# segeschecho/OpenEKFMonoSLAM

Hardware: AMD Instinct MI355X
Metric: EKF updates/s (frames/s) at N features (higher is better)
Workload: dtype f32 storage; i8 MFMA with exact i32 sums (downdate) + f64 (B, S, state)

## Files before the change

### openekfmonoslam_amd/csrc/engine.cpp

```cpp
#include "engine.h"
#include "../../include/ekf_test_hooks.h"

#include <cmath>
#include <cstdio>
#include <algorithm>
#include <atomic>
#include <cstdlib>
#include <chrono>
#include <cstring>
#include <mutex>
#include <new>

#include <dlfcn.h>
#include <rccl/rccl.h>

using namespace ekf;

namespace ekf {
void launch_partition(EkfEngine *e, const EkfMatch *src, int M, const uint8_t *flags, EkfMatch *dst1, EkfMatch *dst0,
                      int *cnt1, bool map_update = false, const uint8_t *d_kdesc = nullptr, int *d_idx0 = nullptr,
                      int publish_seq = 0, bool rescue = false);
void launch_outlier_idx(EkfEngine *e, const EkfMatch *src, int M, int *idx);
}

// ... 573 lines not shown
            if (sharded) {
                sym.resize((size_t)cnt * n);
                for (int i = 0; i < cnt; ++i)
                    for (int j = 0; j < n; ++j) {
                        const double a = P[(size_t)(g0 + i) * n + j], c = P[(size_t)j * n + g0 + i];
                        sym[(size_t)i * n + j] = e->f32 ? (double)(0.5f * (float)a + 0.5f * (float)c) : 0.5 * a + 0.5 * c;
                    }
                src = sym.data();
            }
            uint8_t *dst = (uint8_t *)e->d.P + (size_t)l0 * e->ldP * w;
            if (e->f32) {
                tmp.resize((size_t)cnt * n);
                for (size_t i = 0; i < (size_t)cnt * n; ++i) tmp[i] = (float)src[i];
                HIPCHK(hipMemcpy2D(dst, (size_t)e->ldP * 4, tmp.data(), (size_t)n * 4, (size_t)n * 4, cnt, hipMemcpyHostToDevice));
            } else {
                HIPCHK(hipMemcpy2D(dst, (size_t)e->ldP * 8, src, (size_t)n * 8, (size_t)n * 8, cnt, hipMemcpyHostToDevice));
            }
        }
        e->p_exact_sym = sharded;
    }
    HIPCHK(hipMemset(e->d.pred_vis, 0, (size_t)e->cap * sizeof(int)));
    HIPCHK(hipMemset(e->d.pred_vis_full, 0, (size_t)e->cap * sizeof(int)));
    e->n_step_preds = 0;
    HIPCHK(hipMemset(e->d.feat_times_predicted, 0, (size_t)e->cap * sizeof(unsigned)));
    HIPCHK(hipMemset(e->d.feat_times_matched, 0, (size_t)e->cap * sizeof(unsigned)));
    return EKF_OK;
}

int ekf_get_state(EkfEngine *e, double x13[13], double *feature_pos, double *P)
{
    if (!e) return EKF_ERR_INVALID_ARG;
    HIPCHK(hipSetDevice(e->device));
    HIPCHK(hipStreamSynchronize(e->stream));
    const int pending = take_pending_error(e);
    if (x13) HIPCHK(hipMemcpy(x13, e->d.state, 13 * sizeof(double), hipMemcpyDeviceToHost));
    if (feature_pos && e->N > 0)
        HIPCHK(hipMemcpy(feature_pos, e->d.feat_pos, (size_t)6 * e->N * sizeof(double), hipMemcpyDeviceToHost));
    if (P) {
        const int n = e->n;
        const size_t w = e->f32 ? 4 : 8;
        const bool sharded = e->shard_world > 1;
        const int blocks[2][3] = {{0, sharded ? 13 : n, 0}, {e->rm.r0, sharded ? e->rm.r1 - e->rm.r0 : 0, e->rm.base}};
        std::vector<float> tmp;
        for (const auto &b : blocks) {
            const int g0 = b[0], cnt = b[1], l0 = b[2];
            if (cnt <= 0) continue;
// ... 108 lines not shown
    HIPCHK(hipSetDevice(e->device));
    HIPCHK(hipStreamSynchronize(e->stream));
    HIPCHK(hipMemcpy(preds, e->d.step_preds, (size_t)e->n_step_preds * sizeof(EkfPrediction), hipMemcpyDeviceToHost));
    return EKF_OK;
}

int ekf_get_feature_layout(EkfEngine *e, int32_t *type, int32_t *covpos)
{
    if (!e) return EKF_ERR_INVALID_ARG;
    for (int i = 0; i < e->N; ++i) {
        if (type) type[i] = e->h_type[i];
        if (covpos) covpos[i] = e->h_covpos[i];
    }
    return EKF_OK;
}

int ekf_add_features(EkfEngine *e, const double *uv, const uint8_t *desc32, int count)
{
    if (!e || count < 0 || (count > 0 && !uv)) return EKF_ERR_INVALID_ARG;
    if (count == 0) return EKF_OK;
    NOT_WHEN_SHARDED(e)
    if (e->N + count > e->cap) return EKF_ERR_CAPACITY;
    HIPCHK(hipSetDevice(e->device));
    double *d_uv = e->d.mm_scratch, *d_Jpo = d_uv + 2 * (size_t)e->cap, *d_Jhr = d_Jpo + 42 * (size_t)count;
    HIPCHK(hipMemcpyAsync(d_uv, uv, (size_t)2 * count * sizeof(double), hipMemcpyHostToDevice, e->stream));
    uint8_t *dd = e->d.feat_desc + (size_t)e->N * e->desc_bytes;
    if (desc32) HIPCHK(hipMemcpyAsync(dd, desc32, (size_t)count * e->desc_bytes, hipMemcpyHostToDevice, e->stream));
    else HIPCHK(hipMemsetAsync(dd, 0, (size_t)count * e->desc_bytes, e->stream));
    HIPCHK(hipMemsetAsync(e->d.feat_times_predicted + e->N, 0, (size_t)count * 4, e->stream));
    HIPCHK(hipMemsetAsync(e->d.feat_times_matched + e->N, 0, (size_t)count * 4, e->stream));
    launch_add_features(e, d_uv, count, d_Jpo, d_Jhr);
    for (int j = 0; j < count; ++j) {
        e->h_type.push_back(EKF_FEATURE_INVERSE_DEPTH);
        e->h_covpos.push_back(e->n + 6 * j);
    }
    e->N += count;
    e->n += 6 * count;
    e->n_pred = 0;
    refresh_row_map(e);
    HIPCHK(hipStreamSynchronize(e->stream));
    return check_async(e);
}

static int compact_map(EkfEngine *e, const std::vector<uint8_t> &drop_feature, const std::vector<uint8_t> &drop_row)
{
    NOT_WHEN_SHARDED(e)
// ... 40 lines not shown
        return EKF_ERR_INVALID_ARG;
    }
    if (w > 0) {
        HIPCHK(hipMemcpy(e->d.feat_pos, pos.data(), (size_t)6 * w * 8, hipMemcpyHostToDevice));
        HIPCHK(hipMemcpy(e->d.feat_desc, desc.data(), (size_t)w * e->desc_bytes, hipMemcpyHostToDevice));
        HIPCHK(hipMemcpy(e->d.tmpl, tmpl.data(), (size_t)w * 363, hipMemcpyHostToDevice));
        HIPCHK(hipMemcpy(e->d.feat_times_predicted, tp.data(), (size_t)w * 4, hipMemcpyHostToDevice));
        HIPCHK(hipMemcpy(e->d.feat_times_matched, tm.data(), (size_t)w * 4, hipMemcpyHostToDevice));
        HIPCHK(hipMemcpy(e->d.feat_type, e->h_type.data(), (size_t)w * 4, hipMemcpyHostToDevice));
        HIPCHK(hipMemcpy(e->d.feat_covpos, e->h_covpos.data(), (size_t)w * 4, hipMemcpyHostToDevice));
    }
    e->N = w;
    e->n = n_new;
    refresh_row_map(e);
    e->n_pred = 0;
    return check_async(e);
}

int ekf_remove_features(EkfEngine *e, const int32_t *feat_idx, int count)
{
    if (!e || count < 0 || (count > 0 && !feat_idx)) return EKF_ERR_INVALID_ARG;
    if (count == 0) return EKF_OK;
    HIPCHK(hipSetDevice(e->device));
    std::vector<uint8_t> df(e->N, 0), dr(e->n, 0);
    for (int i = 0; i < count; ++i) {
        const int f = feat_idx[i];
        if (f < 0 || f >= e->N || (i > 0 && feat_idx[i] <= feat_idx[i - 1])) return EKF_ERR_INVALID_ARG;
        df[f] = 1;
        for (int k = 0; k < dims_of(e->h_type[f]); ++k) dr[e->h_covpos[f] + k] = 1;
    }
    return compact_map(e, df, dr);
}

int ekf_remove_bad_features(EkfEngine *e, int *n_removed)
{
    if (!e) return EKF_ERR_INVALID_ARG;
    HIPCHK(hipSetDevice(e->device));
    HIPCHK(hipStreamSynchronize(e->stream));
    const int N = e->N;
    std::vector<unsigned> tp(N), tm(N);
    if (N > 0) {
        HIPCHK(hipMemcpy(tp.data(), e->d.feat_times_predicted, (size_t)N * 4, hipMemcpyDeviceToHost));
        HIPCHK(hipMemcpy(tm.data(), e->d.feat_times_matched, (size_t)N * 4, hipMemcpyDeviceToHost));
    }
    std::vector<int32_t> idx;
    for (int i = 0; i < N; ++i) {
        const float pct = static_cast<float>(tm[i]) / static_cast<float>(tp[i]);
        if (pct < e->cfg.par.goodFeatureMatchingPercent) idx.push_back(i);
    }
    if (n_removed) *n_removed = (int)idx.size();
    return ekf_remove_features(e, idx.data(), (int)idx.size());
}

int ekf_convert_inverse_depth_to_depth(EkfEngine *e, int *converted_index)
{
    if (!e) return EKF_ERR_INVALID_ARG;
    if (converted_index) *converted_index = -1;
    if (e->N == 0) return EKF_OK;
    NOT_WHEN_SHARDED(e)
    HIPCHK(hipSetDevice(e->device));
    double *d_li = e->d.mm_scratch;
    launch_linearity(e, d_li);
    std::vector<double> li(e->N);
    HIPCHK(hipMemcpyAsync(li.data(), d_li, (size_t)e->N * 8, hipMemcpyDeviceToHost, e->stream));
    HIPCHK(hipStreamSynchronize(e->stream));
    int fi = -1;
    for (int i = 0; i < e->N; ++i)
        if (e->h_type[i] == EKF_FEATURE_INVERSE_DEPTH && li[i] < e->cfg.par.inverseDepthLinearityIndexThreshold) {
            fi = i;
            break;
        }
    if (fi < 0) return EKF_OK;
    const int pos = e->h_covpos[fi];
    double *d_J = e->d.mm_scratch + e->cap, *d_T3 = d_J + 32;
    launch_convert(e, fi, pos, d_J, d_T3);
    e->h_type[fi] = EKF_FEATURE_DEPTH;
    std::vector<uint8_t> df(e->N, 0), dr(e->n, 0);
    dr[pos + 3] = dr[pos + 4] = dr[pos + 5] = 1;
    if (converted_index) *converted_index = fi;
    return compact_map(e, df, dr);
}

constexpr int POLL_SECONDS = 20;
// ... 35 lines not shown
            for (int i = 0; i < CNT_COUNT; ++i) e->h_counts[i] = m[i];
            return EKF_OK;
        }
        if ((spin & 0xfffff) == 0xfffff &&
            ((hipStreamQuery(e->stream) == hipSuccess && m[CNT_COUNT] != seq) || std::chrono::steady_clock::now() > t_end)) break;
#if defined(__x86_64__)
        __builtin_ia32_pause();
#endif
    }
    return read_counts(e);
}

static int check_async(EkfEngine *e)
{
    HIPCHK(hipGetLastError());
    return EKF_OK;
}

int ekf_predict(EkfEngine *e)
{
    if (!e) return EKF_ERR_INVALID_ARG;
    HIPCHK(hipSetDevice(e->device));
    launch_predict(e);
    return check_async(e);
}

static int complete_hp_table(EkfEngine *e)
{
    if (e->shard_world <= 1 || e->hp_complete) return EKF_OK;
    int rc;
    std::vector<int32_t> rb(e->shard_world + 1);
    for (int r = 0; r <= e->shard_world; ++r) rb[r] = 2 * e->shard_feat_begin[r];
    if ((rc = exchange_rows(e, EKF_XCHG_HP, e->d.HP, (size_t)e->ldP * hp_elem_bytes(e), rb, "the H.P row blocks"))) return rc;
    if (e->f32 && !e->exact && (rc = exchange_rows(e, EKF_XCHG_HPC, e->d.HPc, 16 * sizeof(double), rb, "the fp64 camera columns of H.P"))) return rc;
    e->hp_complete = true;
    return EKF_OK;
}

static int predict_measurements_dev(EkfEngine *e, const int *d_idx, int count, int *n_out, bool count_predicted = false,
                                    bool lean = false)
{
    launch_predict_features(e, d_idx, d_idx ? count : e->N, false);
    const bool slots = lean && !d_idx && e->shard_world > 1;
    if (slots) launch_shard_bounds_idx(e, e->d.plist, e->d.counts + CNT_NPRED);
    int rc = read_counts(e);
    if (rc) return rc;
    const int np = e->h_counts[d_idx ? CNT_NPRED_SUB : CNT_NPRED];
    if (slots) {
        e->slot_rb.assign(e->shard_world + 1, 0);
        for (int r = 0; r <= e->shard_world; ++r) e->slot_rb[r] = e->h_counts[CNT_SHARD0 + r];
    } else if (!d_idx) e->slot_rb.clear();
    launch_hp_rows(e, d_idx ? e->d.plist_sub : e->d.plist, np, count_predicted);
    if (!d_idx) e->n_pred = np;
    *n_out = np;
    if (e->shard_world > 1 && np > 0) {
        e->hp_complete = false;
        if (!lean && (rc = complete_hp_table(e))) return rc;
        std::vector<int32_t> rb(e->shard_world + 1);
        for (int r = 0; r <= e->shard_world; ++r) rb[r] = e->shard_feat_begin[r];
        if ((rc = exchange_rows(e, EKF_XCHG_PRED_S, e->d.pred_S, 4 * sizeof(double), rb, "the innovation covariance blocks"))) return rc;
    }
    if (!d_idx && e->keep_step_preds) {
        launch_pack_predictions(e, e->d.plist, np, e->d.step_preds);
        e->n_step_preds = np;
    }
    if (!d_idx && e->img.valid) {
        launch_gate_snapshot(e, np);
        e->n_gates = np;
    }
    return check_async(e);
}

static int download_predictions(EkfEngine *e, const int *d_list, int np, EkfPrediction *preds, double *Hs, double *Hf)
{
    if (np <= 0) return EKF_OK;
// ... 183 lines not shown
    int rc = validate_matches(e, matches, M);
    if (rc) return rc;
    if (n_hypotheses) *n_hypotheses = 0;
    if (M == 0) return EKF_OK;
    HIPCHK(hipSetDevice(e->device));
    HIPCHK(hipMemcpyAsync(e->d.matches, matches, (size_t)M * sizeof(EkfMatch), hipMemcpyHostToDevice, e->stream));
    if ((rc = complete_hp_table(e))) return rc;
    rc = ransac_dev(e, M);
    if (rc) return rc;
    HIPCHK(hipMemcpy(inlier_mask, e->d.best_flags, (size_t)M, hipMemcpyDeviceToHost));
    if (n_hypotheses) *n_hypotheses = e->h_counts[CNT_RS_NEXT];
    return EKF_OK;
}

static int lean_gather_exchange(EkfEngine *e, int M)
{
    (void)M;
    int rc;
    if ((rc = exchange_rows(e, EKF_XCHG_HP, e->d.G, (size_t)e->ldP * hp_elem_bytes(e), e->shard_rb, "the gathered H.P rows"))) return rc;
    if (e->f32 && !e->exact && (rc = exchange_rows(e, EKF_XCHG_HPC, e->d.Gc, 16 * sizeof(double), e->shard_rb, "their fp64 camera columns"))) return rc;
    return EKF_OK;
}

static int update_dev(EkfEngine *e, int M, bool update_cov, bool lean = false)
{
    if (M <= 0) return EKF_OK;
    lean = lean && e->shard_world > 1 && !e->hp_complete;
    if (lean) {
        launch_shard_bounds(e, e->d.msel, M);
        int rc = read_counts(e);
        if (rc) return rc;
        e->shard_rb.assign(e->shard_world + 1, 0);
        for (int r = 0; r <= e->shard_world; ++r) e->shard_rb[r] = 2 * e->h_counts[CNT_SHARD0 + r];
        if (e->shard_rb[0] != 0 || e->shard_rb[e->shard_world] != 2 * M) {
            e->err = "sharded update: the match list is not in feature order";
            return EKF_ERR_INVALID_ARG;
        }
    }
    EkfMatch *save = e->d.matches;
    e->d.matches = e->d.msel;
    e->after_gather = lean ? lean_gather_exchange : nullptr;
    launch_update(e, M, update_cov);
    e->after_gather = nullptr;
    e->d.matches = save;
    if (e->hook_rc) return e->hook_rc;
    return check_async(e);
}

static int recover_failed_update(EkfEngine *e, int *status)
// ... 160 lines not shown
static int detect_step_keypoints(EkfEngine *e);

static int step_dev(EkfEngine *e, const EkfKeypoint *d_kps, const uint8_t *d_desc, int n_kp, EkfStepInfo *info,
                    bool use_ncc = false, bool detect = false)
{
    const bool dev_counts = !use_ncc && !detect && !e->img.valid && !e->keep_step_preds && e->shard_world == 1;
    const bool lean = e->shard_world > 1;
    int *cnt = e->d.counts;
    EkfStepInfo li;
    std::memset(&li, 0, sizeof(li));
    int status = EKF_OK, rc;
    const int retries0 = e->sweep_retries;
    if (!dev_counts && e->err_unread) {
        if ((rc = read_counts(e))) return rc;
        if ((rc = recover_failed_update(e, &status))) return rc;
    }
    bool restarted = false;
restart:
    StageTimer tm(e);
    tm.mark();
    int np = 0;
    if (dev_counts) {
        const bool deferred = launch_predict_with_features(e, e->N);
        launch_hp_rows(e, e->d.plist, e->N, true, cnt + CNT_NPRED, deferred);
    } else {
        launch_predict(e);
        if ((rc = predict_measurements_dev(e, nullptr, e->N, &np, true, lean))) return rc;
    }
    tm.mark();
    int M = 0;
    if (dev_counts) {
        launch_match(e, d_kps, d_desc, e->N, n_kp, cnt + CNT_NPRED, true);
    } else {
        if (detect && (rc = detect_step_keypoints(e))) return rc;
        if (lean) rc = match_sharded_dev(e, use_ncc, d_kps, d_desc, n_kp, &M);
        else rc = use_ncc ? match_ncc_dev(e, &M) : match_dev(e, d_kps, d_desc, n_kp, &M, detect ? cnt + CNT_KP_FOUND : nullptr);
        if (rc) return rc;
    }
    tm.mark();
    if (dev_counts) {
        const int batch = e->cfg.ransac_batch;
        const int seq_r = next_publish_seq(e);
        launch_ransac_batch(e, e->N, 0, batch, cnt + CNT_NMATCH, seq_r);
        if ((rc = wait_counts(e, seq_r))) return rc;
        if (e->h_counts[CNT_ERR] && !restarted) {
            if ((rc = recover_failed_update(e, &status))) return rc;
            restarted = true;
// ... 3 lines not shown
        M = e->h_counts[CNT_NMATCH];
        for (int h0 = batch, nb = batch * RANSAC_WIDE_FACTOR; !e->h_counts[CNT_RS_DONE] && h0 < M; h0 += nb) {
            launch_ransac_batch(e, M, h0, nb);
            if ((rc = read_counts(e))) return rc;
        }
    } else if (M > 0 && (rc = ransac_dev(e, M, lean))) {
        return rc;
    }
    li.n_predicted = np;
    li.n_matches = M;
    int ni = 0, no = 0;
    if (M > 0) {
        li.n_hypotheses = e->h_counts[CNT_RS_NEXT];
        ni = e->h_counts[CNT_RS_BEST];
        no = M - ni;
        launch_partition(e, e->d.matches, M, e->d.best_flags, e->d.msel, e->d.mout, nullptr, true, d_desc, e->d.work_idx);
    }
    li.n_inliers = ni;
    li.n_outliers = no;
    tm.mark();
    if ((rc = update_dev(e, ni, true, lean))) return rc;
    tm.mark();
    int nr = 0;
    if (no > 0) {
        int nop = 0;
        for (int attempt = 0; attempt < 2; ++attempt) {
            if (dev_counts) {
                launch_predict_features(e, e->d.work_idx, no, false);
                launch_hp_rows(e, e->d.plist_sub, no, false, cnt + CNT_NPRED_SUB);
                const int seq_p = next_publish_seq(e);
                launch_partition(e, e->d.mout, no, e->d.mask, e->d.msel, nullptr, cnt + CNT_NRESC, true, d_desc, nullptr, seq_p, true);
                rc = wait_counts(e, seq_p);
            } else {
                rc = predict_measurements_dev(e, e->d.work_idx, no, &nop, false, lean);
            }
            if (rc) return rc;
            if (!e->h_counts[CNT_ERR]) break;
            if ((rc = recover_failed_update(e, &status))) return rc;
        }
        if (dev_counts) {
            nr = e->h_counts[CNT_NRESC];
        } else if (nop > 0) {
            launch_rescue(e, e->d.mout, no);
            launch_partition(e, e->d.mout, no, e->d.mask, e->d.msel, nullptr, cnt + CNT_NRESC, true, d_desc);
            if ((rc = read_counts(e))) return rc;
            nr = e->h_counts[CNT_NRESC];
        }
    }
    li.n_rescued = nr;
    tm.mark();
    if ((rc = update_dev(e, nr, true, lean))) return rc;
    tm.mark();
    if (dev_counts && e->async_errors) {
        e->err_unread = true;
    } else {
        if ((rc = read_counts(e))) return rc;
        if (detect) {
            e->step_kp_detected = e->h_counts[CNT_KP_FOUND];
            e->step_kp_kept = std::min(e->step_kp_detected, e->kcap);
        }
        if ((rc = recover_failed_update(e, &status))) return rc;
    }
    tm.finish();
    li.status = status;
    li.n_sweep_retries = e->sweep_retries - retries0;
    if (info) *info = li;
    return status;
}

int ekf_set_async_errors(EkfEngine *e, int on)
{
    if (!e) return EKF_ERR_INVALID_ARG;
    e->async_errors = on != 0;
    return EKF_OK;
// ... 589 lines not shown
```

### openekfmonoslam_amd/csrc/engine.h

```cpp
#pragma once
#include <hip/hip_runtime.h>

#include <atomic>
#include <cstdint>
#include <map>
#include <memory>
#include <mutex>
#include <string>
#include <vector>

#include "../../include/ekf_engine.h"
#include "device_math.h"

namespace ekf {

constexpr int NB = 32;
constexpr int LD_ALIGN = 128;
constexpr int B_SWEEP_MAX = 2048;
constexpr int DX_SPLIT = 16;
constexpr int RANSAC_WIDE_FACTOR = 8;
#ifndef PX_S_VALUE
#define PX_S_VALUE 5
#endif
constexpr int PX_S = PX_S_VALUE;
// ... 154 lines not shown
};

}

struct EkfEngine {
    EkfEngineConfig cfg;
    ekf::CamD cam;
    ekf::ParD par;
    int device = 0;
    int cap = 0, ncap = 0, mcap = 0, kcap = 0;
    int ldP = 0, ldS = 0, ldW = 0;
    int N = 0, n = 0;
    bool f32 = false;
    bool exact = false;
    int desc_bytes = EKF_DESC_BYTES;
    bool desc_f32 = false;
    int shard_rank = 0, shard_world = 1;
    int p_rows_cap = 0;
    ekf::RowMap rm{13, 13, 13};
    std::vector<int> shard_feat_begin;
    EkfExchangeFn xchg = nullptr;
    void *comm = nullptr;
    bool hp_complete = true;
    int (*after_gather)(EkfEngine *, int) = nullptr;
    int (*exchange_hook)(EkfEngine *, int what, void *base, size_t row_bytes, const std::vector<int32_t> &rb, const char *name) = nullptr;
    std::vector<int32_t> shard_row_begin;
    long long xchg_bytes_planes = 0;
    int hook_rc = 0;
    std::vector<int32_t> shard_rb;
    std::vector<int32_t> slot_rb;
    std::vector<int32_t> last_col_rb;
    void *xchg_user = nullptr;
    int n_cus = 256;
    int b_path = 0;
    int sweep_mode = 2;
    unsigned ps_epoch = 0;
    int ps_fault = 0;
    std::shared_ptr<ekf::SweepRegistry> ps_reg;
    int force_launches = 0;
    int sweep_retries = 0;
    int ps_backoff = 0, ps_backoff_len = 0, ps_ok_streak = 0;
    int last_update_M = 0;
    bool last_update_cov = true;
    bool last_update_sym = false;
    bool last_update_persist = false;
    int ps_cap[2] = {0, 0};
// ... 79 lines not shown
    int x = c;
#pragma unroll
    for (int o = 1; o < 64; o <<= 1) {
        const int y = __shfl_up(x, o, 64);
        if (lane >= o) x += y;
    }
    if (lane == 63) wtot[wv] = x;
    __syncthreads();
    int base = 0, tot = 0;
#pragma unroll
    for (int w = 0; w < 16; ++w) {
        const int t = wtot[w];
        base += w < wv ? t : 0;
        tot += t;
    }
    *total = tot;
    return base + x - c;
}
#endif

void launch_predict(EkfEngine *e);
bool launch_predict_features(EkfEngine *e, const int *d_idx, int count, bool state_only, bool defer_compact = false);
bool launch_predict_with_features(EkfEngine *e, int count);
void launch_hp_rows(EkfEngine *e, const int *d_list, int n_list, bool count_predicted = false, const int *d_count = nullptr, bool from_flags = false);
void launch_match(EkfEngine *e, const EkfKeypoint *kps, const uint8_t *kdesc, int n_pred, int n_kp, const int *d_npred = nullptr,
                  bool with_ransac_init = false, const int *d_nkp = nullptr);
void launch_match_index(EkfEngine *e, int M, const int *d_M = nullptr);
void launch_shard_bounds(EkfEngine *e, const EkfMatch *list, int count);
void launch_shard_bounds_idx(EkfEngine *e, const int *list, const int *d_count);
void launch_match_slots(EkfEngine *e, const EkfKeypoint *kps, const uint8_t *kdesc, int n_kp, int s_lo, int s_hi);
void launch_match_ncc_slots(EkfEngine *e, int s_lo, int s_hi);
void launch_match_compact(EkfEngine *e, const EkfKeypoint *kps, int n_pred);
void launch_match_compact_slots(EkfEngine *e, int n_pred, const EkfKeypoint *d_slot_xy);
void launch_ransac_hyp(EkfEngine *e, int M, int h0, int batch, const int *d_M, int h_lo, int h_hi);
void launch_ransac_select(EkfEngine *e, int M, int h0, int batch, const int *d_M, int publish_seq);
void launch_ransac_batch(EkfEngine *e, int M, int h0, int batch, const int *d_M = nullptr, int publish_seq = 0);
void launch_ransac_init(EkfEngine *e, int M);
void launch_update(EkfEngine *e, int M, bool update_cov);
void launch_p_update_exact(EkfEngine *e, int m, bool use_bc, bool exps_ready = false, bool planes_ready = false);
void launch_round_P_f32(EkfEngine *e);
void launch_diag_extract(EkfEngine *e, float *diag);
void launch_planes_move(EkfEngine *e, bool pack, int m_k, int c_lo, int c_hi, int skip_lo, int skip_hi);
void launch_dx_planes(EkfEngine *e, int m_k);
void launch_slice_columns(EkfEngine *e, int m, int c_lo, int c_hi);
void launch_b_gemm_planes(EkfEngine *e, int m, int c_lo, int c_hi);
void launch_rescue(EkfEngine *e, const EkfMatch *matches, int M);
void launch_state_only_predict(EkfEngine *e, EkfPrediction *d_out);
// ... 33 lines not shown
```

### openekfmonoslam_amd/csrc/kernels_predict.hip

```cpp
#include "engine.h"

namespace ekf {

__device__ void predict_prepare_serial(double *st, double *sG);

__global__ void __launch_bounds__(256) k_predict_prepare(double *st, ParD par, const int *counts)
{
    __shared__ double sG[13 * 6];
    if (filter_frozen(counts)) return;
    const double dt = 1.0;
    const double ln = par.linearAccelSD * par.linearAccelSD * dt * dt;
    const double an = par.angularAccelSD * par.angularAccelSD * dt * dt;
    if (blockIdx.x != 0) return;
    if (threadIdx.x == 0) predict_prepare_serial(st, sG);
    __syncthreads();
    if (threadIdx.x < 169) {
        const int i = threadIdx.x / 13, j = threadIdx.x % 13;
        double s = 0.0;
        for (int k = 0; k < 6; ++k) s += (sG[i * 6 + k] * (k < 3 ? ln : an)) * sG[j * 6 + k];
        st[ST_GQG + i * 13 + j] = s;
    }
}

__device__ void predict_prepare_serial(double *st, double *sG)
// ... 247 lines not shown
        return false;
    }
    int *list = sub ? e->d.plist_sub : e->d.plist, *cnt = e->d.counts + (sub ? CNT_NPRED_SUB : CNT_NPRED);
#define PF_ARGS(L_, C_) e->d.state, e->cam, e->d.feat_pos, e->d.feat_type, d_idx, count, e->d.work_flag, state_only ? e->d.pred_vis2 : e->d.pred_vis, \
                        state_only ? e->d.pred_uv2 : e->d.pred_uv, state_only ? nullptr : e->d.Hs, state_only ? nullptr : e->d.Hf,                      \
                        sub ? nullptr : e->d.pred_vis_full, L_, C_
    if (count <= 256) {
        k_predict_features<256><<<1, 256, 0, e->stream>>>(PF_ARGS(list, cnt));
        return false;
    }
    const int nb = (count + 255) / 256;
    k_predict_features<256><<<nb, 256, 0, e->stream>>>(PF_ARGS(nullptr, nullptr));
#undef PF_ARGS
    if (defer_compact && !sub && !d_idx) return true;
    k_compact<<<1, 1024, 0, e->stream>>>(e->d.work_flag, d_idx, count, sub ? e->d.plist_sub : e->d.plist,
                                         e->d.counts + (sub ? CNT_NPRED_SUB : CNT_NPRED));
    return false;
}

template <typename T, typename TO>
__global__ void __launch_bounds__(256)
k_hp_rows(const T *P, int ld, int n, const int *list, const int *feat_type, const int *feat_covpos,
          const double *Hs_tab, const double *Hf_tab, TO *HP, double *S_tab, RowMap rm, double *HPc, unsigned *times_predicted,
          const int *d_count, const int *flag, int n_items, int *list_out, int *count_out, const int *counts)
{
    const int tid = threadIdx.x;
    if (flag) {
        if ((int)blockIdx.x == n_items) {
            if (blockIdx.y != 0) return;
            __shared__ int wtot[16];
            if (tid < 16) wtot[tid] = 0;
            __syncthreads();
            const int per = (n_items + 255) / 256;
            const int b = tid * per, e = min(n_items, b + per);
            int c = 0;
            for (int i = b; i < e; ++i) c += flag[i] ? 1 : 0;
            int total;
            int pos = block_exclusive_scan_1024(c, wtot, &total);
            for (int i = b; i < e; ++i)
                if (flag[i]) list_out[pos++] = i;
            if (tid == 0) *count_out = total;
            return;
        }
        if (!flag[blockIdx.x]) return;
    } else if (d_count && (int)blockIdx.x >= *d_count) return;
    __shared__ double sH[26];
    __shared__ double sHP[2][13];
    const int fi = flag ? (int)blockIdx.x : list[blockIdx.x];
    const int d = feat_dim(feat_type[fi]);
    const int pos = feat_covpos[fi];
    const bool first = blockIdx.y == 0;
    if (times_predicted && tid == 0 && first && !filter_frozen(counts)) times_predicted[fi]++;
    if (!owns_row(rm, pos)) return;
    const T *Pf = P + (size_t)local_row(rm, pos) * ld;
    if (tid < 14) sH[tid] = Hs_tab[14 * fi + tid];
    else if (tid < 26) sH[tid] = Hf_tab[12 * fi + tid - 14];
    double pcol[13];
    int jcol = -1;
    if (first && tid >= 64 && tid < 64 + 7 + d) {
        jcol = tid - 64 < 7 ? tid - 64 : pos + (tid - 64 - 7);
#pragma unroll
        for (int a = 0; a < 6; ++a) pcol[a] = a < d ? (double)Pf[(size_t)a * ld + jcol] : 0.0;
#pragma unroll
        for (int a = 0; a < 7; ++a) pcol[6 + a] = (double)P[(size_t)a * ld + jcol];
    }
    __syncthreads();
    if (jcol >= 0) {
        double a0 = 0.0, a1 = 0.0, b0 = 0.0, b1 = 0.0;
#pragma unroll
        for (int a = 0; a < 6; ++a)
            if (a < d) {
                a0 += sH[14 + a] * pcol[a];
                a1 += sH[20 + a] * pcol[a];
            }
#pragma unroll
        for (int a = 0; a < 7; ++a) {
            b0 += sH[a] * pcol[6 + a];
            b1 += sH[7 + a] * pcol[6 + a];
        }
        sHP[0][tid - 64] = a0 + b0;
        sHP[1][tid - 64] = a1 + b1;
    }
    TO *o0 = HP + (size_t)(2 * fi) * ld;
    TO *o1 = o0 + ld;
    constexpr int VW = 16 / sizeof(T);
    typedef T vec_t __attribute__((ext_vector_type(VW)));
    const int jb = ((int)blockIdx.y * 256 + tid) * VW;
    if (jb < n) {
        vec_t pf[6], pc[7];
#pragma unroll
        for (int a = 0; a < 6; ++a)
            if (a < d) pf[a] = *(const vec_t *)(Pf + (size_t)a * ld + jb);
#pragma unroll
        for (int a = 0; a < 7; ++a) pc[a] = *(const vec_t *)(P + (size_t)a * ld + jb);
        typedef TO ovec_t __attribute__((ext_vector_type(VW)));
        ovec_t r0, r1;
#pragma unroll
        for (int v = 0; v < VW; ++v) {
            const int j = jb + v;
            double a0 = 0.0, a1 = 0.0;
#pragma unroll
            for (int a = 0; a < 6; ++a)
                if (a < d) {
                    const double p = (double)pf[a][v];
                    a0 += sH[14 + a] * p;
                    a1 += sH[20 + a] * p;
                }
            double b0 = 0.0, b1 = 0.0;
#pragma unroll
            for (int a = 0; a < 7; ++a) {
                const double p = (double)pc[a][v];
// ... 9 lines not shown
                HPc[(size_t)(2 * fi + 1) * 16 + j] = a1;
            }
        }
        if (jb + VW <= n) {
            *(ovec_t *)(o0 + jb) = r0;
            *(ovec_t *)(o1 + jb) = r1;
        } else {
#pragma unroll
            for (int v = 0; v < VW; ++v)
                if (jb + v < n) { o0[jb + v] = r0[v]; o1[jb + v] = r1[v]; }
        }
    }
    if (!first) return;
    __syncthreads();
    if (tid < 4) {
        const int r = tid >> 1, c = tid & 1;
        double s1 = 0.0, s2 = 0.0;
        for (int a = 0; a < 7; ++a) s1 += sHP[r][a] * sH[c * 7 + a];
        for (int a = 0; a < d; ++a) s2 += sHP[r][7 + a] * sH[14 + c * 6 + a];
        S_tab[4 * fi + tid] = s1 + s2 + (r == c ? 1.0 : 0.0);
    }
}

void launch_hp_rows(EkfEngine *e, const int *d_list, int n_list, bool count_predicted, const int *d_count, bool from_flags)
{
    unsigned *tp = count_predicted ? e->d.feat_times_predicted : nullptr;
    if (n_list <= 0) return;
    const int chunks_f = (e->n + 256 * 4 - 1) / (256 * 4), chunks_d = (e->n + 256 * 2 - 1) / (256 * 2);
    const int *flag = from_flags ? e->d.work_flag : nullptr;
    int *lo = from_flags ? e->d.plist : nullptr, *co = from_flags ? e->d.counts + CNT_NPRED : nullptr;
    const int gx = n_list + (from_flags ? 1 : 0);
    if (e->exact && e->f32)
        k_hp_rows<float, double><<<dim3(gx, chunks_f), 256, 0, e->stream>>>((const float *)e->d.P, e->ldP, e->n, d_list, e->d.feat_type,
                                                        e->d.feat_covpos, e->d.Hs, e->d.Hf, (double *)e->d.HP,
                                                        e->d.pred_S, e->rm, e->d.HPc, tp, d_count, flag, n_list, lo, co, e->d.counts);
    else if (e->f32)
        k_hp_rows<float, float><<<dim3(gx, chunks_f), 256, 0, e->stream>>>((const float *)e->d.P, e->ldP, e->n, d_list, e->d.feat_type,
                                                        e->d.feat_covpos, e->d.Hs, e->d.Hf, (float *)e->d.HP,
                                                        e->d.pred_S, e->rm, e->d.HPc, tp, d_count, flag, n_list, lo, co, e->d.counts);
    else
        k_hp_rows<double, double><<<dim3(gx, chunks_d), 256, 0, e->stream>>>((const double *)e->d.P, e->ldP, e->n, d_list,
                                                         e->d.feat_type, e->d.feat_covpos, e->d.Hs, e->d.Hf,
                                                         (double *)e->d.HP, e->d.pred_S, e->rm, e->d.HPc, tp, d_count, flag, n_list, lo, co, e->d.counts);
}

__global__ void __launch_bounds__(256)
k_pack_predictions(const int *list, const int *count, const double *uv_tab, const double *S_tab, EkfPrediction *out,
                   int with_S)
{
    const int k = blockIdx.x * 256 + threadIdx.x;
    if (k >= *count) return;
    const int fi = list[k];
    EkfPrediction p;
    p.featureIndex = fi;
    p._pad = 0;
    p.imagePos[0] = uv_tab[2 * fi];
    p.imagePos[1] = uv_tab[2 * fi + 1];
    for (int i = 0; i < 4; ++i) p.covarianceMatrix[i] = with_S ? S_tab[4 * fi + i] : 0.0;
    out[k] = p;
}

__global__ void __launch_bounds__(256)
k_pack_predictions_n(const int *list, int n, const double *uv_tab, const double *S_tab, EkfPrediction *out)
{
    const int k = blockIdx.x * 256 + threadIdx.x;
    if (k >= n) return;
// ... 25 lines not shown
```

### openekfmonoslam_amd/csrc/kernels_ransac.hip

```cpp
#include "engine.h"

namespace ekf {

constexpr int HYP_THREADS = 512;

template <typename T>
__global__ void __launch_bounds__(HYP_THREADS)
k_ransac_hyp(const double *st, CamD cam, double thr, const double *feat_pos, const int *feat_type,
             const int *feat_covpos, int N, const T *HP, int ld, const double *uv_tab, const double *S_tab,
             const EkfMatch *matches, int M, const int *match_of_feat, int h0, int *hyp_count, uint8_t *hyp_flags,
             int mcap, const int *d_M, int h_lo, int h_hi)
{
    __shared__ double sx[13], sRt[9], sRinv[9], sw[2];
    __shared__ int s_cnt[HYP_THREADS / 64];
    if (d_M) M = *d_M;
    const int h = h0 + blockIdx.x;
    if (h >= M) return;
    if (h < h_lo || h >= h_hi) return;
    const int tid = threadIdx.x;
    const int fi = matches[h].featureIndex;
    const T *g0 = HP + (size_t)(2 * fi) * ld;
    const T *g1 = g0 + ld;
    if (tid == 0) {
        double S[4] = {S_tab[4 * fi] - 1.0 + cam.pixelErrorX, S_tab[4 * fi + 1], S_tab[4 * fi + 2],
                       S_tab[4 * fi + 3] - 1.0 + cam.pixelErrorX};
        double Si[4];
        inv2(S, Si);
        const double ax = matches[h].imagePos[0] - uv_tab[2 * fi];
        const double ay = matches[h].imagePos[1] - uv_tab[2 * fi + 1];
        const double n0 = fabs(ax) > EKF_DELTA ? ax : 0.0;
        const double n1 = fabs(ay) > EKF_DELTA ? ay : 0.0;
        const double w0 = Si[0] * n0 + Si[1] * n1;
        const double w1 = Si[2] * n0 + Si[3] * n1;
        sw[0] = w0;
        sw[1] = w1;
        double x[13];
        for (int i = 0; i < 13; ++i) {
            const double dx = (double)g0[i] * w0 + (double)g1[i] * w1;
            x[i] = st[ST_X + i] + (fabs(dx) > EKF_DELTA ? dx : 0.0);
            sx[i] = x[i];
        }
        double R[9];
        quat_to_rot(x + 3, R);
        for (int i = 0; i < 3; ++i)
            for (int j = 0; j < 3; ++j) sRt[j * 3 + i] = R[i * 3 + j];
        inv3(R, sRinv);
    }
    __syncthreads();
    const double w0 = sw[0], w1 = sw[1];
    uint8_t *flags = hyp_flags + (size_t)blockIdx.x * mcap;
    const int nthr = blockDim.x;
    for (int k = tid; k < M; k += nthr) flags[k] = 0;
    __syncthreads();
    int cnt = 0;
    for (int f = tid; f < N; f += nthr) {
        const int mi = match_of_feat[f];
        if (mi >= M) continue;
        const int type = feat_type[f], pos = feat_covpos[f], d = feat_dim(type);
        double fp[6];
        for (int a = 0; a < 6; ++a) fp[a] = feat_pos[6 * f + a];
        for (int a = 0; a < d; ++a) {
            const double dx = (double)g0[pos + a] * w0 + (double)g1[pos + a] * w1;
            if (fabs(dx) > EKF_DELTA) fp[a] += dx;
        }
        double uv[2];
        int ok = 0;
        if (predict_pixel(cam, sx, sRt, sRinv, fp, type, uv)) {
            const double xd = matches[mi].imagePos[0] - uv[0];
            const double yd = matches[mi].imagePos[1] - uv[1];
            ok = sqrt(xd * xd + yd * yd) < thr ? 1 : 0;
        }
        flags[mi] = (uint8_t)ok;
        cnt += ok;
    }
    cnt = wave_sum_i(cnt);
    if ((tid & 63) == 0) s_cnt[tid >> 6] = cnt;
    __syncthreads();
    if (tid == 0) {
        int tot = 0;
        for (int w = 0; w < nthr / 64; ++w) tot += s_cnt[w];
        hyp_count[blockIdx.x] = tot;
    }
}

__global__ void __launch_bounds__(256)
k_ransac_select(int *counts, const int *hyp_count, const uint8_t *hyp_flags, uint8_t *best_flags, int M, int h0,
// ... 42 lines not shown
{
    const int i = blockIdx.x * 256 + threadIdx.x;
    if (i == 0) {
        counts[CNT_RS_BEST] = 0;
        counts[CNT_RS_BESTH] = -1;
        counts[CNT_RS_NHYP] = 1000;
        counts[CNT_RS_NEXT] = 0;
        counts[CNT_RS_DONE] = 0;
    }
    if (i < N) match_of_feat[i] = 0x7fffffff;
    if (i < M) best_flags[i] = 0;
}

void launch_ransac_init(EkfEngine *e, int M)
{
    const int n = max(max(e->N, M), 1);
    k_ransac_init<<<(n + 255) / 256, 256, 0, e->stream>>>(e->d.counts, e->d.match_of_feat, e->d.best_flags, e->N, M);
}

void launch_ransac_hyp(EkfEngine *e, int M, int h0, int batch, const int *d_M, int h_lo, int h_hi)
{
    const int nb = batch;
    const double thr = e->cfg.par.ransacThresholdPredictDistance;
    if (e->f32 && !e->exact)
        k_ransac_hyp<float><<<nb, e->N > 256 ? HYP_THREADS : 256, 0, e->stream>>>(e->d.state, e->cam, thr, e->d.feat_pos, e->d.feat_type,
                                                       e->d.feat_covpos, e->N, (const float *)e->d.HP, e->ldP,
                                                       e->d.pred_uv, e->d.pred_S, e->d.matches, M,
                                                       e->d.match_of_feat, h0, e->d.hyp_count, e->d.hyp_flags,
                                                       e->mcap, d_M, h_lo, h_hi);
    else
        k_ransac_hyp<double><<<nb, e->N > 256 ? HYP_THREADS : 256, 0, e->stream>>>(e->d.state, e->cam, thr, e->d.feat_pos, e->d.feat_type,
                                                        e->d.feat_covpos, e->N, (const double *)e->d.HP, e->ldP,
                                                        e->d.pred_uv, e->d.pred_S, e->d.matches, M,
                                                        e->d.match_of_feat, h0, e->d.hyp_count, e->d.hyp_flags,
                                                        e->mcap, d_M, h_lo, h_hi);
}

void launch_ransac_select(EkfEngine *e, int M, int h0, int batch, const int *d_M, int publish_seq)
{
    k_ransac_select<<<1, 256, 0, e->stream>>>(e->d.counts, e->d.hyp_count, e->d.hyp_flags, e->d.best_flags, M, h0,
                                              batch, e->mcap, e->cfg.par.ransacAllInliersProbability, d_M, e->d_mirror,
                                              e->d_mirror ? publish_seq : 0);
}

void launch_ransac_batch(EkfEngine *e, int M, int h0, int batch, const int *d_M, int publish_seq)
{
    launch_ransac_hyp(e, M, h0, batch, d_M, 0, 0x7fffffff);
    launch_ransac_select(e, M, h0, batch, d_M, publish_seq);
}

__global__ void __launch_bounds__(256)
k_rescue(const EkfMatch *m, int M, const int *vis, const double *uv_tab, const double *S_tab, double chi2,
         uint8_t *mask)
{
    const int i = blockIdx.x * 256 + threadIdx.x;
    if (i >= M) return;
    const int fi = m[i].featureIndex;
    const double d0 = m[i].imagePos[0] - uv_tab[2 * fi];
// ... 18 lines not shown
```

Measured before the change: 1206.

## Defer full HP row formation to matched features and compute RANSAC gains from P

In the device-count step path, the per-predicted-feature HP row kernel now computes only S (s_only) rather than full HP rows over all n columns. RANSAC hypotheses recompute the few HP elements they need directly from P and the H tables, and full HP rows are built only for matched features just before the update, tracked with a validity flag. This is meant to drop the O(N·n) HP construction for unmatched predictions, at the cost of repeated per-hypothesis P reads and added invalidation bookkeeping.

```diff
diff --git a/openekfmonoslam_amd/csrc/engine.cpp b/openekfmonoslam_amd/csrc/engine.cpp
--- a/openekfmonoslam_amd/csrc/engine.cpp
+++ b/openekfmonoslam_amd/csrc/engine.cpp
@@ -619,6 +619,7 @@
     HIPCHK(hipMemset(e->d.pred_vis, 0, (size_t)e->cap * sizeof(int)));
     HIPCHK(hipMemset(e->d.pred_vis_full, 0, (size_t)e->cap * sizeof(int)));
     e->n_step_preds = 0;
+    e->hp_table_valid = false;
     HIPCHK(hipMemset(e->d.feat_times_predicted, 0, (size_t)e->cap * sizeof(unsigned)));
     HIPCHK(hipMemset(e->d.feat_times_matched, 0, (size_t)e->cap * sizeof(unsigned)));
     return EKF_OK;
@@ -773,6 +774,7 @@
     NOT_WHEN_SHARDED(e)
     if (e->N + count > e->cap) return EKF_ERR_CAPACITY;
     HIPCHK(hipSetDevice(e->device));
+    e->hp_table_valid = false;
     double *d_uv = e->d.mm_scratch, *d_Jpo = d_uv + 2 * (size_t)e->cap, *d_Jhr = d_Jpo + 42 * (size_t)count;
     HIPCHK(hipMemcpyAsync(d_uv, uv, (size_t)2 * count * sizeof(double), hipMemcpyHostToDevice, e->stream));
     uint8_t *dd = e->d.feat_desc + (size_t)e->N * e->desc_bytes;
@@ -859,6 +861,7 @@
     if (!e || count < 0 || (count > 0 && !feat_idx)) return EKF_ERR_INVALID_ARG;
     if (count == 0) return EKF_OK;
     HIPCHK(hipSetDevice(e->device));
+    e->hp_table_valid = false;
     std::vector<uint8_t> df(e->N, 0), dr(e->n, 0);
     for (int i = 0; i < count; ++i) {
         const int f = feat_idx[i];
@@ -873,6 +876,7 @@
 {
     if (!e) return EKF_ERR_INVALID_ARG;
     HIPCHK(hipSetDevice(e->device));
+    e->hp_table_valid = false;
     HIPCHK(hipStreamSynchronize(e->stream));
     const int N = e->N;
     std::vector<unsigned> tp(N), tm(N);
@@ -896,6 +900,7 @@
     if (e->N == 0) return EKF_OK;
     NOT_WHEN_SHARDED(e)
     HIPCHK(hipSetDevice(e->device));
+    e->hp_table_valid = false;
     double *d_li = e->d.mm_scratch;
     launch_linearity(e, d_li);
     std::vector<double> li(e->N);
@@ -977,6 +982,7 @@
     if (!e) return EKF_ERR_INVALID_ARG;
     HIPCHK(hipSetDevice(e->device));
     launch_predict(e);
+    e->hp_table_valid = false;
     return check_async(e);
 }
 
@@ -1006,6 +1012,7 @@
         for (int r = 0; r <= e->shard_world; ++r) e->slot_rb[r] = e->h_counts[CNT_SHARD0 + r];
     } else if (!d_idx) e->slot_rb.clear();
     launch_hp_rows(e, d_idx ? e->d.plist_sub : e->d.plist, np, count_predicted);
+    if (!d_idx) e->hp_table_valid = true;
     if (!d_idx) e->n_pred = np;
     *n_out = np;
     if (e->shard_world > 1 && np > 0) {
@@ -1235,9 +1242,11 @@
     return EKF_OK;
 }
 
-static int update_dev(EkfEngine *e, int M, bool update_cov, bool lean = false)
+static int update_dev(EkfEngine *e, int M, bool update_cov, bool lean = false, bool rows_formed = false)
 {
     if (M <= 0) return EKF_OK;
+    if (e->shard_world == 1 && !e->hp_table_valid && !rows_formed) launch_hp_rows_matches(e, e->d.msel, M);
+    if (update_cov) e->hp_table_valid = false;
     lean = lean && e->shard_world > 1 && !e->hp_complete;
     if (lean) {
         launch_shard_bounds(e, e->d.msel, M);
@@ -1444,7 +1453,8 @@
     int np = 0;
     if (dev_counts) {
         const bool deferred = launch_predict_with_features(e, e->N);
-        launch_hp_rows(e, e->d.plist, e->N, true, cnt + CNT_NPRED, deferred);
+        e->hp_table_valid = false;
+        launch_hp_rows(e, e->d.plist, e->N, true, cnt + CNT_NPRED, deferred, true);
     } else {
         launch_predict(e);
         if ((rc = predict_measurements_dev(e, nullptr, e->N, &np, true, lean))) return rc;
@@ -1494,6 +1504,7 @@
     if ((rc = update_dev(e, ni, true, lean))) return rc;
     tm.mark();
     int nr = 0;
+    bool rows_current = no > 0;
     if (no > 0) {
         int nop = 0;
         for (int attempt = 0; attempt < 2; ++attempt) {
@@ -1509,6 +1520,7 @@
             if (rc) return rc;
             if (!e->h_counts[CNT_ERR]) break;
             if ((rc = recover_failed_update(e, &status))) return rc;
+            rows_current = attempt == 0;
         }
         if (dev_counts) {
             nr = e->h_counts[CNT_NRESC];
@@ -1521,7 +1533,7 @@
     }
     li.n_rescued = nr;
     tm.mark();
-    if ((rc = update_dev(e, nr, true, lean))) return rc;
+    if ((rc = update_dev(e, nr, true, lean, rows_current))) return rc;
     tm.mark();
     if (dev_counts && e->async_errors) {
         e->err_unread = true;
diff --git a/openekfmonoslam_amd/csrc/engine.h b/openekfmonoslam_amd/csrc/engine.h
--- a/openekfmonoslam_amd/csrc/engine.h
+++ b/openekfmonoslam_amd/csrc/engine.h
@@ -200,6 +200,7 @@
     EkfExchangeFn xchg = nullptr;
     void *comm = nullptr;
     bool hp_complete = true;
+    bool hp_table_valid = false;
     int (*after_gather)(EkfEngine *, int) = nullptr;
     int (*exchange_hook)(EkfEngine *, int what, void *base, size_t row_bytes, const std::vector<int32_t> &rb, const char *name) = nullptr;
     std::vector<int32_t> shard_row_begin;
@@ -325,7 +326,9 @@
 void launch_predict(EkfEngine *e);
 bool launch_predict_features(EkfEngine *e, const int *d_idx, int count, bool state_only, bool defer_compact = false);
 bool launch_predict_with_features(EkfEngine *e, int count);
-void launch_hp_rows(EkfEngine *e, const int *d_list, int n_list, bool count_predicted = false, const int *d_count = nullptr, bool from_flags = false);
+void launch_hp_rows(EkfEngine *e, const int *d_list, int n_list, bool count_predicted = false, const int *d_count = nullptr, bool from_flags = false,
+                    bool s_only = false, const EkfMatch *mlist = nullptr);
+void launch_hp_rows_matches(EkfEngine *e, const EkfMatch *matches, int M);
 void launch_match(EkfEngine *e, const EkfKeypoint *kps, const uint8_t *kdesc, int n_pred, int n_kp, const int *d_npred = nullptr,
                   bool with_ransac_init = false, const int *d_nkp = nullptr);
 void launch_match_index(EkfEngine *e, int M, const int *d_M = nullptr);
diff --git a/openekfmonoslam_amd/csrc/kernels_predict.hip b/openekfmonoslam_amd/csrc/kernels_predict.hip
--- a/openekfmonoslam_amd/csrc/kernels_predict.hip
+++ b/openekfmonoslam_amd/csrc/kernels_predict.hip
@@ -293,7 +293,8 @@
 __global__ void __launch_bounds__(256)
 k_hp_rows(const T *P, int ld, int n, const int *list, const int *feat_type, const int *feat_covpos,
           const double *Hs_tab, const double *Hf_tab, TO *HP, double *S_tab, RowMap rm, double *HPc, unsigned *times_predicted,
-          const int *d_count, const int *flag, int n_items, int *list_out, int *count_out, const int *counts)
+          const int *d_count, const int *flag, int n_items, int *list_out, int *count_out, const int *counts, int s_only,
+          const EkfMatch *mlist)
 {
     const int tid = threadIdx.x;
     if (flag) {
@@ -317,10 +318,10 @@
     } else if (d_count && (int)blockIdx.x >= *d_count) return;
     __shared__ double sH[26];
     __shared__ double sHP[2][13];
-    const int fi = flag ? (int)blockIdx.x : list[blockIdx.x];
+    const int fi = flag ? (int)blockIdx.x : (mlist ? mlist[blockIdx.x].featureIndex : list[blockIdx.x]);
     const int d = feat_dim(feat_type[fi]);
     const int pos = feat_covpos[fi];
-    const bool first = blockIdx.y == 0;
+    const bool first = blockIdx.y == 0 && !mlist;
     if (times_predicted && tid == 0 && first && !filter_frozen(counts)) times_predicted[fi]++;
     if (!owns_row(rm, pos)) return;
     const T *Pf = P + (size_t)local_row(rm, pos) * ld;
@@ -357,7 +358,7 @@
     constexpr int VW = 16 / sizeof(T);
     typedef T vec_t __attribute__((ext_vector_type(VW)));
     const int jb = ((int)blockIdx.y * 256 + tid) * VW;
-    if (jb < n) {
+    if (!s_only && jb < n) {
         vec_t pf[6], pc[7];
 #pragma unroll
         for (int a = 0; a < 6; ++a)
@@ -413,26 +414,32 @@
     }
 }
 
-void launch_hp_rows(EkfEngine *e, const int *d_list, int n_list, bool count_predicted, const int *d_count, bool from_flags)
+void launch_hp_rows(EkfEngine *e, const int *d_list, int n_list, bool count_predicted, const int *d_count, bool from_flags, bool s_only,
+                    const EkfMatch *mlist)
 {
     unsigned *tp = count_predicted ? e->d.feat_times_predicted : nullptr;
     if (n_list <= 0) return;
-    const int chunks_f = (e->n + 256 * 4 - 1) / (256 * 4), chunks_d = (e->n + 256 * 2 - 1) / (256 * 2);
+    const int chunks_f = s_only ? 1 : (e->n + 256 * 4 - 1) / (256 * 4), chunks_d = s_only ? 1 : (e->n + 256 * 2 - 1) / (256 * 2);
     const int *flag = from_flags ? e->d.work_flag : nullptr;
     int *lo = from_flags ? e->d.plist : nullptr, *co = from_flags ? e->d.counts + CNT_NPRED : nullptr;
     const int gx = n_list + (from_flags ? 1 : 0);
+#define HP_TAIL e->d.pred_S, e->rm, e->d.HPc, tp, d_count, flag, n_list, lo, co, e->d.counts, s_only ? 1 : 0, mlist
     if (e->exact && e->f32)
         k_hp_rows<float, double><<<dim3(gx, chunks_f), 256, 0, e->stream>>>((const float *)e->d.P, e->ldP, e->n, d_list, e->d.feat_type,
-                                                        e->d.feat_covpos, e->d.Hs, e->d.Hf, (double *)e->d.HP,
-                                                        e->d.pred_S, e->rm, e->d.HPc, tp, d_count, flag, n_list, lo, co, e->d.counts);
+                                                        e->d.feat_covpos, e->d.Hs, e->d.Hf, (double *)e->d.HP, HP_TAIL);
     else if (e->f32)
         k_hp_rows<float, float><<<dim3(gx, chunks_f), 256, 0, e->stream>>>((const float *)e->d.P, e->ldP, e->n, d_list, e->d.feat_type,
-                                                        e->d.feat_covpos, e->d.Hs, e->d.Hf, (float *)e->d.HP,
-                                                        e->d.pred_S, e->rm, e->d.HPc, tp, d_count, flag, n_list, lo, co, e->d.counts);
+                                                        e->d.feat_covpos, e->d.Hs, e->d.Hf, (float *)e->d.HP, HP_TAIL);
     else
         k_hp_rows<double, double><<<dim3(gx, chunks_d), 256, 0, e->stream>>>((const double *)e->d.P, e->ldP, e->n, d_list,
                                                          e->d.feat_type, e->d.feat_covpos, e->d.Hs, e->d.Hf,
-                                                         (double *)e->d.HP, e->d.pred_S, e->rm, e->d.HPc, tp, d_count, flag, n_list, lo, co, e->d.counts);
+                                                         (double *)e->d.HP, HP_TAIL);
+#undef HP_TAIL
+}
+
+void launch_hp_rows_matches(EkfEngine *e, const EkfMatch *matches, int M)
+{
+    launch_hp_rows(e, nullptr, M, false, nullptr, false, false, matches);
 }
 
 __global__ void __launch_bounds__(256)
diff --git a/openekfmonoslam_amd/csrc/kernels_ransac.hip b/openekfmonoslam_amd/csrc/kernels_ransac.hip
--- a/openekfmonoslam_amd/csrc/kernels_ransac.hip
+++ b/openekfmonoslam_amd/csrc/kernels_ransac.hip
@@ -4,14 +4,42 @@
 
 constexpr int HYP_THREADS = 512;
 
-template <typename T>
+template <typename T, typename TP>
+__device__ __forceinline__ void hp_element(const TP *P, const TP *Pf, int ld, int d, const double *sH, int j, double *g0, double *g1)
+{
+    double pf[6], pc[7];
+#pragma unroll
+    for (int a = 0; a < 6; ++a) pf[a] = a < d ? (double)Pf[(size_t)a * ld + j] : 0.0;
+#pragma unroll
+    for (int a = 0; a < 7; ++a) pc[a] = (double)P[(size_t)a * ld + j];
+    double a0 = 0.0, a1 = 0.0;
+#pragma unroll
+    for (int a = 0; a < 6; ++a)
+        if (a < d) {
+            a0 += sH[14 + a] * pf[a];
+            a1 += sH[20 + a] * pf[a];
+        }
+    double b0 = 0.0, b1 = 0.0;
+#pragma unroll
+    for (int a = 0; a < 7; ++a) {
+        b0 += sH[a] * pc[a];
+        b1 += sH[7 + a] * pc[a];
+    }
+    a0 += b0;
+    a1 += b1;
+    *g0 = (double)(T)a0;
+    *g1 = (double)(T)a1;
+}
+
+template <typename T, typename TP, bool FROM_P>
 __global__ void __launch_bounds__(HYP_THREADS)
 k_ransac_hyp(const double *st, CamD cam, double thr, const double *feat_pos, const int *feat_type,
              const int *feat_covpos, int N, const T *HP, int ld, const double *uv_tab, const double *S_tab,
              const EkfMatch *matches, int M, const int *match_of_feat, int h0, int *hyp_count, uint8_t *hyp_flags,
-             int mcap, const int *d_M, int h_lo, int h_hi)
+             int mcap, const int *d_M, int h_lo, int h_hi, const TP *P, const double *Hs_tab, const double *Hf_tab)
 {
     __shared__ double sx[13], sRt[9], sRinv[9], sw[2];
+    __shared__ double sH[26], sg[2][13];
     __shared__ int s_cnt[HYP_THREADS / 64];
     if (d_M) M = *d_M;
     const int h = h0 + blockIdx.x;
@@ -21,6 +49,15 @@
     const int fi = matches[h].featureIndex;
     const T *g0 = HP + (size_t)(2 * fi) * ld;
     const T *g1 = g0 + ld;
+    const int dh = feat_dim(feat_type[fi]);
+    const TP *Pf = FROM_P ? P + (size_t)feat_covpos[fi] * ld : nullptr;
+    if (FROM_P) {
+        if (tid < 14) sH[tid] = Hs_tab[14 * fi + tid];
+        else if (tid < 26) sH[tid] = Hf_tab[12 * fi + tid - 14];
+        __syncthreads();
+        if (tid < 13) hp_element<T, TP>(P, Pf, ld, dh, sH, tid, &sg[0][tid], &sg[1][tid]);
+        __syncthreads();
+    }
     if (tid == 0) {
         double S[4] = {S_tab[4 * fi] - 1.0 + cam.pixelErrorX, S_tab[4 * fi + 1], S_tab[4 * fi + 2],
                        S_tab[4 * fi + 3] - 1.0 + cam.pixelErrorX};
@@ -36,7 +73,7 @@
         sw[1] = w1;
         double x[13];
         for (int i = 0; i < 13; ++i) {
-            const double dx = (double)g0[i] * w0 + (double)g1[i] * w1;
+            const double dx = FROM_P ? sg[0][i] * w0 + sg[1][i] * w1 : (double)g0[i] * w0 + (double)g1[i] * w1;
             x[i] = st[ST_X + i] + (fabs(dx) > EKF_DELTA ? dx : 0.0);
             sx[i] = x[i];
         }
@@ -59,9 +96,21 @@
         const int type = feat_type[f], pos = feat_covpos[f], d = feat_dim(type);
         double fp[6];
         for (int a = 0; a < 6; ++a) fp[a] = feat_pos[6 * f + a];
-        for (int a = 0; a < d; ++a) {
-            const double dx = (double)g0[pos + a] * w0 + (double)g1[pos + a] * w1;
-            if (fabs(dx) > EKF_DELTA) fp[a] += dx;
+        double ga[6], gb[6];
+        if (FROM_P) {
+#pragma unroll
+            for (int a = 0; a < 6; ++a) hp_element<T, TP>(P, Pf, ld, dh, sH, pos + min(a, d - 1), &ga[a], &gb[a]);
+        } else {
+#pragma unroll
+            for (int a = 0; a < 6; ++a) {
+                ga[a] = (double)g0[pos + min(a, d - 1)];
+                gb[a] = (double)g1[pos + min(a, d - 1)];
+            }
+        }
+#pragma unroll
+        for (int a = 0; a < 6; ++a) {
+            const double dx = ga[a] * w0 + gb[a] * w1;
+            if (a < d && fabs(dx) > EKF_DELTA) fp[a] += dx;
         }
         double uv[2];
         int ok = 0;
@@ -150,18 +199,22 @@
 {
     const int nb = batch;
     const double thr = e->cfg.par.ransacThresholdPredictDistance;
-    if (e->f32 && !e->exact)
-        k_ransac_hyp<float><<<nb, e->N > 256 ? HYP_THREADS : 256, 0, e->stream>>>(e->d.state, e->cam, thr, e->d.feat_pos, e->d.feat_type,
-                                                       e->d.feat_covpos, e->N, (const float *)e->d.HP, e->ldP,
-                                                       e->d.pred_uv, e->d.pred_S, e->d.matches, M,
-                                                       e->d.match_of_feat, h0, e->d.hyp_count, e->d.hyp_flags,
-                                                       e->mcap, d_M, h_lo, h_hi);
-    else
-        k_ransac_hyp<double><<<nb, e->N > 256 ? HYP_THREADS : 256, 0, e->stream>>>(e->d.state, e->cam, thr, e->d.feat_pos, e->d.feat_type,
-                                                        e->d.feat_covpos, e->N, (const double *)e->d.HP, e->ldP,
-                                                        e->d.pred_uv, e->d.pred_S, e->d.matches, M,
-                                                        e->d.match_of_feat, h0, e->d.hyp_count, e->d.hyp_flags,
-                                                        e->mcap, d_M, h_lo, h_hi);
+    const int nt = e->N > 256 ? HYP_THREADS : 256;
+    const bool from_p = e->shard_world == 1 && !e->hp_table_valid;
+#define HYP_ARGS(T_, TP_) e->d.state, e->cam, thr, e->d.feat_pos, e->d.feat_type, e->d.feat_covpos, e->N, (const T_ *)e->d.HP, e->ldP, e->d.pred_uv, \
+                          e->d.pred_S, e->d.matches, M, e->d.match_of_feat, h0, e->d.hyp_count, e->d.hyp_flags, e->mcap, d_M, h_lo, h_hi,          \
+                          (const TP_ *)e->d.P, e->d.Hs, e->d.Hf
+    if (e->f32 && !e->exact) {
+        if (from_p) k_ransac_hyp<float, float, true><<<nb, nt, 0, e->stream>>>(HYP_ARGS(float, float));
+        else k_ransac_hyp<float, float, false><<<nb, nt, 0, e->stream>>>(HYP_ARGS(float, float));
+    } else if (e->f32) {
+        if (from_p) k_ransac_hyp<double, float, true><<<nb, nt, 0, e->stream>>>(HYP_ARGS(double, float));
+        else k_ransac_hyp<double, float, false><<<nb, nt, 0, e->stream>>>(HYP_ARGS(double, float));
+    } else {
+        if (from_p) k_ransac_hyp<double, double, true><<<nb, nt, 0, e->stream>>>(HYP_ARGS(double, double));
+        else k_ransac_hyp<double, double, false><<<nb, nt, 0, e->stream>>>(HYP_ARGS(double, double));
+    }
+#undef HYP_ARGS
 }
 
 void launch_ransac_select(EkfEngine *e, int M, int h0, int batch, const int *d_M, int publish_seq)
```

New measurement: 1215, median of 3. No clear change (+0.8%).
